# Plonky3/Plonky3-recursion

Hardware: AMD Instinct MI355X
Metric: prove_next_layer ms + Poseidon2 perms/s, KoalaBear 2^20-row circuit, 1/8 GPU (lower is better)
Workload: dtype u32 Montgomery (31-bit prime field, degree-4 extension); Poseidon2 hashing as exact integers in f64; 1 GPU; prove_next_layer (verifier-circuit run on the device + prove_all_tables) of the synthetic koala-bear 2^20-row recursion layer: tables const/public/alu/poseidon2/recompose, FRI blowup 4, arity<=4, 54 queries, 15-bit PoW; circuit inputs + NextLayerPrepCache resident in HBM; field=koala-bear, log_height=20, independent_proofs=1, proof_bytes=612900, parallelism=1 independent proofs, one per GPU, no data-path collective

## Files before the change

### plonky3_recursion_amd/csrc/poseidon2_f64.hip.h

```cpp
#pragma once
#include "poseidon2.h"

#if defined(__FAST_MATH__) || defined(__FINITE_MATH_ONLY__) && __FINITE_MATH_ONLY__
#error "poseidon2_f64.hip.h relies on exact IEEE-754 double arithmetic (error-free products, magic-number rounding): do not build with -ffast-math / -Ofast"
#endif

namespace p3r {

template <class PP>
struct P2F64 {
  static constexpr double P = (double)PP::P;
  static constexpr double INVP = 1.0 / (double)PP::P;
  static constexpr double MAGIC = 0x1.8p52;
  static constexpr double P_HI = (double)(PP::P - 1);
};
#pragma clang fp contract(off)

template <class PP>
__device__ __forceinline__ double p2f_quot(double x) {
  return __builtin_fma(x, P2F64<PP>::INVP, P2F64<PP>::MAGIC) - P2F64<PP>::MAGIC;
}

template <class PP>
__device__ __forceinline__ double p2f_reduce(double x) {
  const double q = p2f_quot<PP>(x);
  return __builtin_fma(-q, P2F64<PP>::P, x);
}
template <class PP>
__device__ __forceinline__ double p2f_mul_2exp_neg(double x, double m) {
  const double t = x * m;
  const double f = __builtin_amdgcn_fract(t);
  return __builtin_fma(-f, P2F64<PP>::P, t);
}
template <class PP>
__device__ __forceinline__ double p2f_mul_2exp_neg_add(double x, double m, double a) {
  const double t = __builtin_fma(x, m, a);
  const double f = __builtin_amdgcn_fract(t);
  return __builtin_fma(-f, P2F64<PP>::P, t);
}

template <class PP>
struct P2FSboxK {
  double k, p_hi, magic;
};
template <class PP>
__device__ __forceinline__ P2FSboxK<PP> p2f_sbox_consts() {
  P2FSboxK<PP> K;
  K.k = -(P2F64<PP>::MAGIC * P2F64<PP>::P);
  K.p_hi = P2F64<PP>::P_HI;
  K.magic = P2F64<PP>::MAGIC;
  asm volatile("" : "+v"(K.k), "+s"(K.p_hi), "+s"(K.magic));
  return K;
}
template <class PP>
__device__ __forceinline__ double p2f_mulmod_k(double a, double b, double c, const P2FSboxK<PP>& K) {
  const double qm = __builtin_fma(a, c, K.magic);
  const double t = __builtin_fma(qm, K.p_hi, K.k);
  const double e = __builtin_fma(a, b, -t);
  return e - qm;
}

template <class PP>
__device__ __forceinline__ double p2f_sbox(double x, const P2FSboxK<PP>& K) {
  const double c = x * P2F64<PP>::INVP;
  const double x2 = p2f_mulmod_k<PP>(x, x, c, K);
  const double x3 = p2f_mulmod_k<PP>(x2, x, c, K);
  if (PP::SBOX_DEGREE == 3) return x3;
  const double x6 = p2f_mulmod_k<PP>(x3, x3, x3 * P2F64<PP>::INVP, K);
  return p2f_mulmod_k<PP>(x6, x, c, K);
}

__device__ __forceinline__ void p2f_mat4(double& x0, double& x1, double& x2, double& x3) {
  const double t01 = x0 + x1, t23 = x2 + x3;
  const double t0123 = t01 + t23;
  const double t01123 = t0123 + x1;
  const double t01233 = t0123 + x3;
  const double n3 = __builtin_fma(x0, 2.0, t01233);
  const double n1 = __builtin_fma(x2, 2.0, t01123);
  const double n0 = t01123 + t01;
  const double n2 = t01233 + t23;
  x0 = n0; x1 = n1; x2 = n2; x3 = n3;
}
__device__ __forceinline__ void p2f_external_linear(double* s) {
#pragma unroll
  for (int i = 0; i < P2_WIDTH; i += 4) p2f_mat4(s[i], s[i + 1], s[i + 2], s[i + 3]);
  double sum[4];
#pragma unroll
  for (int k = 0; k < 4; ++k) sum[k] = (s[k] + s[4 + k]) + (s[8 + k] + s[12 + k]);
#pragma unroll
  for (int i = 0; i < P2_WIDTH; ++i) s[i] += sum[i & 3];
}

template <class PP>
struct P2FDiag {
  double three, a, b, c, d;
};
template <class PP>
__device__ __forceinline__ P2FDiag<PP> p2f_diag_consts() {
  P2FDiag<PP> k;
  k.three = 3.0;
  k.a = 0x1p-8;
  k.b = PP::FIELD_ID == 0 ? 0x1p-3 : 0x1p-2;
  k.c = PP::FIELD_ID == 0 ? 0x1p-4 : 0x1p-3;
  k.d = PP::FIELD_ID == 0 ? 0x1p-24 : 0x1p-4;
  asm volatile("" : "+s"(k.three), "+s"(k.a), "+s"(k.b), "+s"(k.c), "+s"(k.d));
  return k;
}

template <class PP>
__device__ __forceinline__ void p2f_internal_linear(double* s, bool reduce_wide, const P2FDiag<PP>& K) {
  if (reduce_wide) {
    s[2] = p2f_reduce<PP>(s[2]);
    s[4] = p2f_reduce<PP>(s[4]);
    s[5] = p2f_reduce<PP>(s[5]);
    s[7] = p2f_reduce<PP>(s[7]);
    s[8] = p2f_reduce<PP>(s[8]);
  }
  double part = ((s[1] + s[2]) + (s[3] + s[4])) + ((s[5] + s[6]) + (s[7] + s[8]));
  part += ((s[9] + s[10]) + (s[11] + s[12])) + ((s[13] + s[14]) + s[15]);
  const double sum = p2f_reduce<PP>(part + s[0]);
  s[0] = __builtin_fma(s[0], -2.0, sum);
  s[1] = s[1] + sum;
  s[2] = __builtin_fma(s[2], 2.0, sum);
  s[3] = p2f_mul_2exp_neg_add<PP>(s[3], 0.5, sum);
  s[4] = __builtin_fma(s[4], K.three, sum);
  s[5] = __builtin_fma(s[5], 4.0, sum);
  s[6] = p2f_mul_2exp_neg_add<PP>(s[6], -0.5, sum);
  s[7] = __builtin_fma(s[7], -K.three, sum);
  s[8] = __builtin_fma(s[8], -4.0, sum);
  s[9] = p2f_mul_2exp_neg_add<PP>(s[9], K.a, sum);
  if (PP::FIELD_ID == 0) {
    s[10] = p2f_mul_2exp_neg_add<PP>(s[10], K.b, sum);
    s[11] = p2f_mul_2exp_neg<PP>(s[11], K.d) + sum;
    s[12] = p2f_mul_2exp_neg_add<PP>(s[12], -K.a, sum);
    s[13] = p2f_mul_2exp_neg_add<PP>(s[13], -K.b, sum);
    s[14] = p2f_mul_2exp_neg_add<PP>(s[14], -K.c, sum);
    s[15] = p2f_mul_2exp_neg<PP>(s[15], -K.d) + sum;
  } else {
    s[10] = p2f_mul_2exp_neg_add<PP>(s[10], K.b, sum);
    s[11] = p2f_mul_2exp_neg_add<PP>(s[11], K.c, sum);
    s[12] = p2f_mul_2exp_neg<PP>(s[12], 0x1p-27) + sum;
    s[13] = p2f_mul_2exp_neg_add<PP>(s[13], -K.a, sum);
    s[14] = p2f_mul_2exp_neg_add<PP>(s[14], -K.d, sum);
    s[15] = p2f_mul_2exp_neg<PP>(s[15], -0x1p-27) + sum;
  }
}

template <class PP, unsigned CARRIED = 0xFFFFu>
__device__ __forceinline__ void p2f_permute(double* s, const double* __restrict__ rc) {
  const P2FSboxK<PP> SK = p2f_sbox_consts<PP>();
#pragma unroll
  for (int i = 0; i < P2_WIDTH; ++i)
    if (CARRIED >> i & 1u) s[i] = p2f_reduce<PP>(s[i]);
  p2f_external_linear(s);
  int k = 0;
#pragma unroll 2
  for (int r = 0; r < P2_HALF_FULL; ++r) {
#pragma unroll
    for (int i = 0; i < P2_WIDTH; ++i) s[i] = p2f_sbox<PP>(s[i] + rc[k + i], SK);
    k += P2_WIDTH;
    p2f_external_linear(s);
  }
  const P2FDiag<PP> K = p2f_diag_consts<PP>();
  for (int r = 0; r < PP::PARTIAL_ROUNDS; ++r) {
    s[0] = p2f_sbox<PP>(s[0] + rc[k + r], SK);
    p2f_internal_linear<PP>(s, r == 6 || r == 15, K);
  }
  k += PP::PARTIAL_ROUNDS;
  s[2] = p2f_reduce<PP>(s[2]);
  s[4] = p2f_reduce<PP>(s[4]);
  s[5] = p2f_reduce<PP>(s[5]);
  s[7] = p2f_reduce<PP>(s[7]);
  s[8] = p2f_reduce<PP>(s[8]);
#pragma unroll 2
  for (int r = 0; r < P2_HALF_FULL; ++r) {
#pragma unroll
    for (int i = 0; i < P2_WIDTH; ++i) s[i] = p2f_sbox<PP>(s[i] + rc[k + i], SK);
    k += P2_WIDTH;
    p2f_external_linear(s);
  }
}

template <class PP>
__device__ __forceinline__ double p2f_load(uint32_t mont) {
  using F = Fp<PP>;
  return (double)F::reduce64_lazy((uint64_t)mont);
}
template <class PP>
__device__ __forceinline__ uint32_t p2f_store(double x) {
  const double r = p2f_reduce<PP>(x * 0x1p32);
  const int32_t v = (int32_t)r;
  return (uint32_t)(v + ((v >> 31) & (int32_t)PP::P));
}

#pragma clang fp contract(fast)

}
```

Measured before the change: 28.23 ms.

## Schedule lazy reductions per lane across fully unrolled Poseidon2 partial rounds

Replaces the generic per-round internal linear layer with a compile-time per-lane schedule. Each lane has a form (integer multiplier, dyadic fraction, or wrap) and reduces modulo p only on rounds chosen so values stay exact in FP64. Dyadic lanes are summed separately and get one fract-based fixup only when needed. A constexpr bound walk checked by static_assert proves the schedule stays exact. The partial rounds are fully unrolled via integer_sequence and the helpers are made host/device, which removes most of the per-round fract/reduce work at the cost of a larger instruction stream and more register pressure.

```diff
diff --git a/plonky3_recursion_amd/csrc/poseidon2_f64.hip.h b/plonky3_recursion_amd/csrc/poseidon2_f64.hip.h
--- a/plonky3_recursion_amd/csrc/poseidon2_f64.hip.h
+++ b/plonky3_recursion_amd/csrc/poseidon2_f64.hip.h
@@ -1,4 +1,6 @@
 #pragma once
+#include <utility>
+
 #include "poseidon2.h"
 
 #if defined(__FAST_MATH__) || defined(__FINITE_MATH_ONLY__) && __FINITE_MATH_ONLY__
@@ -17,25 +19,33 @@
 #pragma clang fp contract(off)
 
 template <class PP>
-__device__ __forceinline__ double p2f_quot(double x) {
+P3R_HD double p2f_quot(double x) {
   return __builtin_fma(x, P2F64<PP>::INVP, P2F64<PP>::MAGIC) - P2F64<PP>::MAGIC;
 }
 
-template <class PP>
-__device__ __forceinline__ double p2f_reduce(double x) {
+P3R_HD double p2f_fract(double x) {
+#if defined(__HIP_DEVICE_COMPILE__)
+  return __builtin_amdgcn_fract(x);
+#else
+  return x - __builtin_floor(x);
+#endif
+}
+
+template <class PP>
+P3R_HD double p2f_reduce(double x) {
   const double q = p2f_quot<PP>(x);
   return __builtin_fma(-q, P2F64<PP>::P, x);
 }
 template <class PP>
-__device__ __forceinline__ double p2f_mul_2exp_neg(double x, double m) {
+P3R_HD double p2f_mul_2exp_neg(double x, double m) {
   const double t = x * m;
-  const double f = __builtin_amdgcn_fract(t);
+  const double f = p2f_fract(t);
   return __builtin_fma(-f, P2F64<PP>::P, t);
 }
 template <class PP>
-__device__ __forceinline__ double p2f_mul_2exp_neg_add(double x, double m, double a) {
+P3R_HD double p2f_mul_2exp_neg_add(double x, double m, double a) {
   const double t = __builtin_fma(x, m, a);
-  const double f = __builtin_amdgcn_fract(t);
+  const double f = p2f_fract(t);
   return __builtin_fma(-f, P2F64<PP>::P, t);
 }
 
@@ -44,16 +54,18 @@
   double k, p_hi, magic;
 };
 template <class PP>
-__device__ __forceinline__ P2FSboxK<PP> p2f_sbox_consts() {
+P3R_HD P2FSboxK<PP> p2f_sbox_consts() {
   P2FSboxK<PP> K;
   K.k = -(P2F64<PP>::MAGIC * P2F64<PP>::P);
   K.p_hi = P2F64<PP>::P_HI;
   K.magic = P2F64<PP>::MAGIC;
+#if defined(__HIP_DEVICE_COMPILE__)
   asm volatile("" : "+v"(K.k), "+s"(K.p_hi), "+s"(K.magic));
+#endif
   return K;
 }
 template <class PP>
-__device__ __forceinline__ double p2f_mulmod_k(double a, double b, double c, const P2FSboxK<PP>& K) {
+P3R_HD double p2f_mulmod_k(double a, double b, double c, const P2FSboxK<PP>& K) {
   const double qm = __builtin_fma(a, c, K.magic);
   const double t = __builtin_fma(qm, K.p_hi, K.k);
   const double e = __builtin_fma(a, b, -t);
@@ -61,7 +73,7 @@
 }
 
 template <class PP>
-__device__ __forceinline__ double p2f_sbox(double x, const P2FSboxK<PP>& K) {
+P3R_HD double p2f_sbox(double x, const P2FSboxK<PP>& K) {
   const double c = x * P2F64<PP>::INVP;
   const double x2 = p2f_mulmod_k<PP>(x, x, c, K);
   const double x3 = p2f_mulmod_k<PP>(x2, x, c, K);
@@ -70,7 +82,7 @@
   return p2f_mulmod_k<PP>(x6, x, c, K);
 }
 
-__device__ __forceinline__ void p2f_mat4(double& x0, double& x1, double& x2, double& x3) {
+P3R_HD void p2f_mat4(double& x0, double& x1, double& x2, double& x3) {
   const double t01 = x0 + x1, t23 = x2 + x3;
   const double t0123 = t01 + t23;
   const double t01123 = t0123 + x1;
@@ -81,7 +93,7 @@
   const double n2 = t01233 + t23;
   x0 = n0; x1 = n1; x2 = n2; x3 = n3;
 }
-__device__ __forceinline__ void p2f_external_linear(double* s) {
+P3R_HD void p2f_external_linear(double* s) {
 #pragma unroll
   for (int i = 0; i < P2_WIDTH; i += 4) p2f_mat4(s[i], s[i + 1], s[i + 2], s[i + 3]);
   double sum[4];
@@ -91,63 +103,217 @@
   for (int i = 0; i < P2_WIDTH; ++i) s[i] += sum[i & 3];
 }
 
-template <class PP>
-struct P2FDiag {
-  double three, a, b, c, d;
+enum P2FForm : int { P2F_SBOX, P2F_INT, P2F_DYADIC, P2F_WRAP };
+struct P2FLane {
+  int form;
+  int d;
+  int k;
+  int first, every;
 };
 template <class PP>
-__device__ __forceinline__ P2FDiag<PP> p2f_diag_consts() {
-  P2FDiag<PP> k;
-  k.three = 3.0;
-  k.a = 0x1p-8;
-  k.b = PP::FIELD_ID == 0 ? 0x1p-3 : 0x1p-2;
-  k.c = PP::FIELD_ID == 0 ? 0x1p-4 : 0x1p-3;
-  k.d = PP::FIELD_ID == 0 ? 0x1p-24 : 0x1p-4;
-  asm volatile("" : "+s"(k.three), "+s"(k.a), "+s"(k.b), "+s"(k.c), "+s"(k.d));
-  return k;
-}
-
-template <class PP>
-__device__ __forceinline__ void p2f_internal_linear(double* s, bool reduce_wide, const P2FDiag<PP>& K) {
-  if (reduce_wide) {
-    s[2] = p2f_reduce<PP>(s[2]);
-    s[4] = p2f_reduce<PP>(s[4]);
-    s[5] = p2f_reduce<PP>(s[5]);
-    s[7] = p2f_reduce<PP>(s[7]);
-    s[8] = p2f_reduce<PP>(s[8]);
-  }
-  double part = ((s[1] + s[2]) + (s[3] + s[4])) + ((s[5] + s[6]) + (s[7] + s[8]));
-  part += ((s[9] + s[10]) + (s[11] + s[12])) + ((s[13] + s[14]) + s[15]);
-  const double sum = p2f_reduce<PP>(part + s[0]);
-  s[0] = __builtin_fma(s[0], -2.0, sum);
-  s[1] = s[1] + sum;
-  s[2] = __builtin_fma(s[2], 2.0, sum);
-  s[3] = p2f_mul_2exp_neg_add<PP>(s[3], 0.5, sum);
-  s[4] = __builtin_fma(s[4], K.three, sum);
-  s[5] = __builtin_fma(s[5], 4.0, sum);
-  s[6] = p2f_mul_2exp_neg_add<PP>(s[6], -0.5, sum);
-  s[7] = __builtin_fma(s[7], -K.three, sum);
-  s[8] = __builtin_fma(s[8], -4.0, sum);
-  s[9] = p2f_mul_2exp_neg_add<PP>(s[9], K.a, sum);
-  if (PP::FIELD_ID == 0) {
-    s[10] = p2f_mul_2exp_neg_add<PP>(s[10], K.b, sum);
-    s[11] = p2f_mul_2exp_neg<PP>(s[11], K.d) + sum;
-    s[12] = p2f_mul_2exp_neg_add<PP>(s[12], -K.a, sum);
-    s[13] = p2f_mul_2exp_neg_add<PP>(s[13], -K.b, sum);
-    s[14] = p2f_mul_2exp_neg_add<PP>(s[14], -K.c, sum);
-    s[15] = p2f_mul_2exp_neg<PP>(s[15], -K.d) + sum;
+constexpr P2FLane p2f_lane(int i) {
+  constexpr P2FLane kb[P2_WIDTH] = {
+      {P2F_SBOX, -2, 0, -1, 0}, {P2F_INT, 1, 0, -1, 0},   {P2F_INT, 2, 0, 10, 0},    {P2F_DYADIC, 1, 1, 9, 10},
+      {P2F_INT, 3, 0, 9, 0},    {P2F_INT, 4, 0, 6, 8},    {P2F_DYADIC, -1, 1, 9, 10}, {P2F_INT, -3, 0, 10, 0},
+      {P2F_INT, -4, 0, 7, 8},   {P2F_DYADIC, 1, 8, 1, 2}, {P2F_DYADIC, 1, 3, 4, 5},   {P2F_WRAP, -127, 0, 1, 3},
+      {P2F_DYADIC, -1, 8, 1, 2}, {P2F_DYADIC, -1, 3, 4, 5}, {P2F_DYADIC, -1, 4, 3, 4}, {P2F_WRAP, 127, 0, 1, 3}};
+  constexpr P2FLane bb[P2_WIDTH] = {
+      {P2F_SBOX, -2, 0, -1, 0}, {P2F_INT, 1, 0, -1, 0},   {P2F_INT, 2, 0, -1, 0},     {P2F_DYADIC, 1, 1, -1, 0},
+      {P2F_INT, 3, 0, 6, 0},    {P2F_INT, 4, 0, 6, 0},    {P2F_DYADIC, -1, 1, -1, 0}, {P2F_INT, -3, 0, 7, 0},
+      {P2F_INT, -4, 0, 7, 0},   {P2F_DYADIC, 1, 8, 0, 2}, {P2F_DYADIC, 1, 2, 6, 6},   {P2F_DYADIC, 1, 3, 5, 7},
+      {P2F_WRAP, -15, 0, 4, 4}, {P2F_DYADIC, -1, 8, 0, 2}, {P2F_DYADIC, -1, 4, 2, 5}, {P2F_WRAP, 15, 0, 4, 4}};
+  return PP::FIELD_ID == 0 ? kb[i] : bb[i];
+}
+template <class PP>
+constexpr bool p2f_lane_hits(int i, int r) {
+  const P2FLane L = p2f_lane<PP>(i);
+  if (L.form == P2F_DYADIC && r == PP::PARTIAL_ROUNDS - 1) return true;
+  if (L.form == P2F_SBOX || L.first < 0 || r < L.first) return false;
+  return L.every == 0 ? r == L.first : (r - L.first) % L.every == 0;
+}
+template <class PP>
+constexpr bool p2f_lane_reduce_after(int i) {
+  const P2FLane L = p2f_lane<PP>(i);
+  return (L.form == P2F_INT || L.form == P2F_WRAP) && L.d != 1 && !p2f_lane_hits<PP>(i, PP::PARTIAL_ROUNDS - 1);
+}
+template <class PP>
+constexpr int p2f_lane_denom(int i, int r) {
+  const P2FLane L = p2f_lane<PP>(i);
+  if (L.form != P2F_DYADIC) return 0;
+  int last = -1;
+  for (int j = 0; j < r; ++j)
+    if (p2f_lane_hits<PP>(i, j)) last = j;
+  return L.k * (r - 1 - last);
+}
+template <class PP>
+constexpr int p2f_frac_denom(int r) {
+  int m = 0;
+  for (int i = 0; i < P2_WIDTH; ++i) m = p2f_lane_denom<PP>(i, r) > m ? p2f_lane_denom<PP>(i, r) : m;
+  return m;
+}
+template <class PP>
+constexpr double p2f_lane_factor(int i) {
+  const P2FLane L = p2f_lane<PP>(i);
+  if (L.form != P2F_DYADIC) return (double)L.d;
+  double m = 1.0;
+  for (int j = 0; j < L.k; ++j) m *= 0.5;
+  return L.d < 0 ? -m : m;
+}
+constexpr double p2f_abs(double x) { return x < 0 ? -x : x; }
+template <class PP>
+constexpr bool p2f_lane_inline(int i) {
+  const double a = p2f_abs(p2f_lane_factor<PP>(i));
+  return a == 0.5 || a == 1.0 || a == 2.0 || a == 4.0;
+}
+template <class PP>
+constexpr int p2f_lane_rep(int i) {
+  for (int j = 0; j < i; ++j)
+    if (p2f_abs(p2f_lane_factor<PP>(j)) == p2f_abs(p2f_lane_factor<PP>(i))) return j;
+  return i;
+}
+template <class PP, int I>
+P3R_HD void p2f_pin_factor(double* mk) {
+  if constexpr (p2f_lane_rep<PP>(I) == I && !p2f_lane_inline<PP>(I)) {
+    mk[I] = p2f_abs(p2f_lane_factor<PP>(I));
+#if defined(__HIP_DEVICE_COMPILE__)
+    asm volatile("" : "+s"(mk[I]));
+#endif
+  }
+}
+
+template <class PP>
+constexpr int p2f_partial_walk() {
+  using u64 = unsigned long long;
+  constexpr u64 EXACT = u64(1) << 53, SBOX_IN = u64(1) << 38, P = PP::P;
+  constexpr u64 SBOX_OUT = (7 * P + 9) / 10, RED = P / 2 + 2;
+  u64 M[P2_WIDTH] = {};
+  int m[P2_WIDTH] = {};
+  for (int i = 0; i < P2_WIDTH; ++i) M[i] = 35 * SBOX_OUT;
+  for (int r = 0; r < PP::PARTIAL_ROUNDS; ++r) {
+    const int at = 1000 * (r + 1);
+    if (M[0] + (P - 1) >= SBOX_IN) return at + 1;
+    M[0] = SBOX_OUT;
+    for (int i = 0; i < P2_WIDTH; ++i) {
+      const P2FLane L = p2f_lane<PP>(i);
+      if ((L.form == P2F_INT || L.form == P2F_WRAP) && p2f_lane_hits<PP>(i, r)) {
+        if (M[i] >= EXACT) return at + 10 * i + 2;
+        M[i] = RED;
+      }
+    }
+    u64 I = 0, F = 0;
+    int mF = 0;
+    for (int i = 0; i < P2_WIDTH; ++i) {
+      if (p2f_lane<PP>(i).form == P2F_DYADIC) {
+        F += M[i];
+        mF = m[i] > mF ? m[i] : mF;
+        if (m[i] != p2f_lane_denom<PP>(i, r)) return at + 10 * i + 3;
+      } else {
+        I += M[i];
+      }
+    }
+    if (mF != p2f_frac_denom<PP>(r) || mF > PP::TWO_ADICITY) return at + 4;
+    if (I >= EXACT || F >= (EXACT >> mF)) return at + 5;
+    const u64 Fi = mF > 0 ? F + P : F;
+    if (I + Fi >= EXACT) return at + 6;
+    const u64 S = RED;
+    for (int i = 0; i < P2_WIDTH; ++i) {
+      const P2FLane L = p2f_lane<PP>(i);
+      if (L.form == P2F_DYADIC) {
+        M[i] = ((M[i] + (u64(1) << L.k) - 1) >> L.k) + S;
+        m[i] += L.k;
+        if (M[i] >= (EXACT >> m[i])) return at + 10 * i + 7;
+        if (p2f_lane_hits<PP>(i, r)) {
+          if (m[i] > PP::TWO_ADICITY || M[i] + P >= EXACT) return at + 10 * i + 8;
+          M[i] += P;
+          m[i] = 0;
+        }
+      } else {
+        M[i] = u64(L.d < 0 ? -L.d : L.d) * M[i] + S;
+        if (M[i] >= EXACT) return at + 10 * i + 9;
+      }
+    }
+  }
+  for (int i = 0; i < P2_WIDTH; ++i) {
+    if (p2f_lane_reduce_after<PP>(i)) M[i] = RED;
+    if (m[i] != 0 || M[i] + (P - 1) >= SBOX_IN) return 100000 + 10 * i;
+  }
+  if (35 * SBOX_OUT >= (u64(1) << 36)) return 100001;
+  return 0;
+}
+static_assert(p2f_partial_walk<KoalaBearParams>() == 0, "KoalaBear: the partial-round schedule leaves exact FP64 arithmetic");
+static_assert(p2f_partial_walk<BabyBearParams>() == 0, "BabyBear: the partial-round schedule leaves exact FP64 arithmetic");
+
+struct P2FLaneList {
+  int n;
+  int lane[P2_WIDTH];
+};
+template <class PP>
+constexpr P2FLaneList p2f_lane_list(bool dyadic) {
+  P2FLaneList l = {0, {}};
+  for (int i = 0; i < P2_WIDTH; ++i)
+    if ((p2f_lane<PP>(i).form == P2F_DYADIC) == dyadic) l.lane[l.n++] = i;
+  return l;
+}
+template <class PP, bool DYADIC>
+P3R_HD double p2f_lane_sum(const double* s) {
+  constexpr P2FLaneList L = p2f_lane_list<PP>(DYADIC);
+  double v[P2_WIDTH];
+#pragma unroll
+  for (int i = 0; i < L.n; ++i) v[i] = s[L.lane[i]];
+#pragma unroll
+  for (int w = 1; w < L.n; w *= 2)
+#pragma unroll
+    for (int i = 0; i + w < L.n; i += 2 * w) v[i] += v[i + w];
+  return v[0];
+}
+
+template <class PP, int R, int I>
+P3R_HD void p2f_lane_reduce(double* s) {
+  constexpr P2FLane L = p2f_lane<PP>(I);
+  if constexpr ((L.form == P2F_INT || L.form == P2F_WRAP) && p2f_lane_hits<PP>(I, R)) s[I] = p2f_reduce<PP>(s[I]);
+}
+template <class PP, int I>
+P3R_HD void p2f_lane_reduce_last(double* s) {
+  if constexpr (p2f_lane_reduce_after<PP>(I)) s[I] = p2f_reduce<PP>(s[I]);
+}
+template <class PP, int R, int I>
+P3R_HD void p2f_lane_diag(double* s, const double* mk, double sum) {
+  constexpr P2FLane L = p2f_lane<PP>(I);
+  constexpr double lit = p2f_lane_factor<PP>(I);
+  constexpr bool inl = p2f_lane_inline<PP>(I);
+  constexpr int rep = p2f_lane_rep<PP>(I);
+  constexpr bool fix = L.form == P2F_DYADIC && p2f_lane_hits<PP>(I, R);
+  const double m = inl ? lit : lit < 0 ? -mk[rep] : mk[rep];
+  if constexpr (lit == 1.0) {
+    s[I] = s[I] + sum;
+  } else if constexpr (fix) {
+    const double t = __builtin_fma(s[I], m, sum);
+    s[I] = __builtin_fma(-p2f_fract(t), P2F64<PP>::P, t);
   } else {
-    s[10] = p2f_mul_2exp_neg_add<PP>(s[10], K.b, sum);
-    s[11] = p2f_mul_2exp_neg_add<PP>(s[11], K.c, sum);
-    s[12] = p2f_mul_2exp_neg<PP>(s[12], 0x1p-27) + sum;
-    s[13] = p2f_mul_2exp_neg_add<PP>(s[13], -K.a, sum);
-    s[14] = p2f_mul_2exp_neg_add<PP>(s[14], -K.d, sum);
-    s[15] = p2f_mul_2exp_neg<PP>(s[15], -0x1p-27) + sum;
-  }
+    s[I] = __builtin_fma(s[I], m, sum);
+  }
+}
+template <class PP, int R, int... I>
+P3R_HD void p2f_partial_round(double* s, const double* __restrict__ rc, const P2FSboxK<PP>& SK, const double* mk,
+                              std::integer_sequence<int, I...>) {
+  s[0] = p2f_sbox<PP>(s[0] + rc[R], SK);
+  (p2f_lane_reduce<PP, R, I>(s), ...);
+  double frac = p2f_lane_sum<PP, true>(s);
+  if constexpr (p2f_frac_denom<PP>(R) > 0) frac = __builtin_fma(-p2f_fract(frac), P2F64<PP>::P, frac);
+  const double sum = p2f_reduce<PP>(p2f_lane_sum<PP, false>(s) + frac);
+  (p2f_lane_diag<PP, R, I>(s, mk, sum), ...);
+}
+template <class PP, int... R, int... I>
+P3R_HD void p2f_partial_rounds(double* s, const double* __restrict__ rc, const P2FSboxK<PP>& SK,
+                               std::integer_sequence<int, R...>, std::integer_sequence<int, I...> lanes) {
+  double mk[P2_WIDTH];
+  (p2f_pin_factor<PP, I>(mk), ...);
+  (p2f_partial_round<PP, R>(s, rc, SK, mk, lanes), ...);
+  (p2f_lane_reduce_last<PP, I>(s), ...);
 }
 
 template <class PP, unsigned CARRIED = 0xFFFFu>
-__device__ __forceinline__ void p2f_permute(double* s, const double* __restrict__ rc) {
+P3R_HD void p2f_permute(double* s, const double* __restrict__ rc) {
   const P2FSboxK<PP> SK = p2f_sbox_consts<PP>();
 #pragma unroll
   for (int i = 0; i < P2_WIDTH; ++i)
@@ -161,17 +327,9 @@
     k += P2_WIDTH;
     p2f_external_linear(s);
   }
-  const P2FDiag<PP> K = p2f_diag_consts<PP>();
-  for (int r = 0; r < PP::PARTIAL_ROUNDS; ++r) {
-    s[0] = p2f_sbox<PP>(s[0] + rc[k + r], SK);
-    p2f_internal_linear<PP>(s, r == 6 || r == 15, K);
-  }
+  p2f_partial_rounds<PP>(s, rc + k, SK, std::make_integer_sequence<int, PP::PARTIAL_ROUNDS>(),
+                         std::make_integer_sequence<int, P2_WIDTH>());
   k += PP::PARTIAL_ROUNDS;
-  s[2] = p2f_reduce<PP>(s[2]);
-  s[4] = p2f_reduce<PP>(s[4]);
-  s[5] = p2f_reduce<PP>(s[5]);
-  s[7] = p2f_reduce<PP>(s[7]);
-  s[8] = p2f_reduce<PP>(s[8]);
 #pragma unroll 2
   for (int r = 0; r < P2_HALF_FULL; ++r) {
 #pragma unroll
@@ -182,12 +340,12 @@
 }
 
 template <class PP>
-__device__ __forceinline__ double p2f_load(uint32_t mont) {
+P3R_HD double p2f_load(uint32_t mont) {
   using F = Fp<PP>;
   return (double)F::reduce64_lazy((uint64_t)mont);
 }
 template <class PP>
-__device__ __forceinline__ uint32_t p2f_store(double x) {
+P3R_HD uint32_t p2f_store(double x) {
   const double r = p2f_reduce<PP>(x * 0x1p32);
   const int32_t v = (int32_t)r;
   return (uint32_t)(v + ((v >> 31) & (int32_t)PP::P));
```

After: 27.18 ms (median of 6 runs). 1.04x faster.
